# iammadab/zk

Measured on AMD Instinct MI355X. Metric: field-ops/sec (MLE fold, 2^24 evals, BN254 Fr) + sumcheck prover wall-clock, higher is better.
Workload: dtype u256 (8 x u32 Montgomery limbs, integer)

## Files before the change

include/zk_amd.h:

```cpp
#ifndef ZK_AMD_H
#define ZK_AMD_H

#include <stddef.h>
#include <stdint.h>

#ifdef __cplusplus
extern "C" {
#endif

#define ZK_AMD_ABI_VERSION 6

typedef enum zk_field {
    ZK_FIELD_BN254_FR = 0,
    ZK_FIELD_BLS12_381_FR = 1,
    ZK_FIELD_BLS12_377_FR = 2
} zk_field;

typedef enum zk_status {
    ZK_OK = 0,
    ZK_ERR_EVAL_LEN = -1,
    ZK_ERR_EVAL_ARITY = -2,
    ZK_ERR_EMPTY_PRODUCT = -3,
    ZK_ERR_ARITY_MISMATCH = -4,
    ZK_ERR_PANIC_INDEX = -5,
// ... 216 lines not shown
int32_t zk_merkle_n_vars(const zk_merkle *m, uint32_t *out);
int32_t zk_merkle_n_columns(const zk_merkle *m, uint32_t *out);
int32_t zk_merkle_root(zk_ctx *ctx, const zk_merkle *m, uint8_t out[32]);
int32_t zk_merkle_level(zk_ctx *ctx, const zk_merkle *m, uint32_t level, uint8_t *out);
int32_t zk_merkle_open(zk_ctx *ctx, const zk_merkle *m, const zk_mle *const *columns, uint32_t n_columns,
                       const uint64_t *indices, uint64_t n_queries, uint64_t *out_rows, uint8_t *out_paths);
int32_t zk_merkle_verify_host(int32_t field, const uint8_t root[32], uint32_t n_vars, uint32_t n_columns, uint64_t index,
                              const uint64_t *row, const uint8_t *path, int32_t *out_ok);

int32_t zk_fri_lde(zk_ctx *ctx, const zk_upoly *p, uint32_t log_n, const uint64_t shift[4], zk_mle **out);
int32_t zk_fri_fold(zk_ctx *ctx, const zk_mle *in, uint32_t log_arity, const uint64_t shift[4], const uint64_t beta[4], zk_mle *out);
int32_t zk_fri_proof_bytes(uint32_t log_degree, uint32_t log_blowup, uint32_t log_arity, uint32_t log_final, uint32_t n_queries, uint64_t *out);
int32_t zk_fri_prove(zk_ctx *ctx, const zk_upoly *p, uint32_t log_degree, uint32_t log_blowup, uint32_t log_arity, uint32_t log_final,
                     uint32_t n_queries, const uint64_t shift[4], const uint8_t seed[32], uint8_t *out_proof);
int32_t zk_fri_verify_host(int32_t field, uint32_t log_degree, uint32_t log_blowup, uint32_t log_arity, uint32_t log_final,
                           uint32_t n_queries, const uint64_t shift[4], const uint8_t seed[32], const uint8_t *proof, uint64_t proof_len,
                           int32_t *out_ok);

typedef struct zk_pcs zk_pcs;
int32_t zk_deep_quotient(zk_ctx *ctx, const zk_mle *const *columns, uint32_t n_columns, const uint64_t shift[4], const uint64_t z[4],
                         const uint64_t *values, const uint64_t alpha[4], zk_mle *out);
int32_t zk_pcs_commit(zk_ctx *ctx, const zk_upoly *const *polys, uint32_t k, uint32_t log_degree, uint32_t log_blowup, uint32_t log_arity,
                      const uint64_t shift[4], zk_pcs **out);
int32_t zk_pcs_free(zk_pcs *h);
int32_t zk_pcs_n_polys(const zk_pcs *h, uint32_t *out);
int32_t zk_pcs_root(zk_ctx *ctx, const zk_pcs *h, uint8_t out[32]);
int32_t zk_pcs_proof_bytes(uint32_t k, uint32_t log_degree, uint32_t log_blowup, uint32_t log_arity, uint32_t log_final, uint32_t n_queries,
                           uint64_t *out);
int32_t zk_pcs_open(zk_ctx *ctx, const zk_pcs *h, const uint64_t z[4], uint32_t log_final, uint32_t n_queries, const uint8_t seed[32],
                    uint64_t *out_values, uint8_t *out_proof);
int32_t zk_pcs_verify_host(int32_t field, uint32_t k, uint32_t log_degree, uint32_t log_blowup, uint32_t log_arity, uint32_t log_final,
                           uint32_t n_queries, const uint64_t shift[4], const uint8_t seed[32], const uint8_t root[32], const uint64_t z[4],
                           const uint64_t *values, const uint8_t *proof, uint64_t proof_len, int32_t *out_ok);

int32_t zk_bench_fold(zk_ctx *ctx, const zk_mle *t, const uint64_t r[4], zk_mle *out, int32_t reps, double *out_ms);
int32_t zk_bench_fold_samples(zk_ctx *ctx, const zk_mle *t, const uint64_t r[4], zk_mle *out, int32_t reps, int32_t group,
                              double *out_ms_each);
int32_t zk_bench_ntt(zk_ctx *ctx, const zk_mle *in, int32_t inverse, zk_mle *out, int32_t reps, double *out_ms);
int32_t zk_bench_upoly_interp(zk_ctx *ctx, const zk_upoly *xs, const zk_upoly *ys, int32_t reps, double *out_ms);
int32_t zk_bench_upoly_evaluate_many(zk_ctx *ctx, const zk_upoly *p, const zk_upoly *xs, int32_t path, int32_t reps, double *out_ms);
int32_t zk_bench_upoly_divrem(zk_ctx *ctx, const zk_upoly *a, const zk_upoly *b, int32_t path, int32_t reps, double *out_ms);
int32_t zk_bench_cmle(zk_ctx *ctx, int32_t op, const zk_mle *t, const zk_cmle *p, const uint64_t *point, uint64_t n_point, int32_t reps,
                      double *out_ms);
int32_t zk_bench_cmle_algebra(zk_ctx *ctx, int32_t op, const zk_cmle *a, const zk_cmle *b, const uint8_t *selectors,
                              const uint64_t *selector_lens, const uint64_t *values, uint64_t n_assign, int32_t reps, double *out_ms);
int32_t zk_bench_batch_inverse(zk_ctx *ctx, const zk_mle *t, zk_mle *out, int32_t path, int32_t reps, double *out_ms);
int32_t zk_bench_merkle(zk_ctx *ctx, const zk_mle *const *columns, uint32_t n_columns, int32_t path, int32_t reps, double *out_ms);
int32_t zk_bench_fri_fold(zk_ctx *ctx, const zk_mle *in, uint32_t log_arity, zk_mle *out, int32_t path, int32_t reps, double *out_ms);
int32_t zk_bench_deep_quotient(zk_ctx *ctx, const zk_mle *const *columns, uint32_t n_columns, zk_mle *out, int32_t reps, double *out_ms);
int32_t zk_bench_prove_partial(zk_ctx *ctx, zk_mle *const *factors, uint64_t k, uint32_t max_var_degree, const uint64_t sum[4],
                               int32_t reps, double *out_ms_each);
int32_t zk_bench_evaluate(zk_ctx *ctx, const zk_mle *t, const uint64_t *point, uint64_t n_point, int32_t reps, double *out_ms_each);
int32_t zk_bench_evaluate_device(zk_ctx *ctx, const zk_mle *t, const uint64_t *point, uint64_t n_point, int32_t reps, double *out_ms);
int32_t zk_bench_modmul(zk_ctx *ctx, int32_t variant, int32_t iters, double *out_modmul_per_s);
int32_t zk_bench_copy(zk_ctx *ctx, uint64_t bytes, int32_t reps, double *out_gbps);


#ifdef __cplusplus
}
#endif
#endif
```

zk_amd/_lib.py:

```python
import ctypes
import os
import re

_HERE = os.path.dirname(os.path.abspath(__file__))
_DEFAULT_LIB = os.path.join(_HERE, "libzk_amd.so")
LIB_PATH = os.environ.get("ZK_AMD_LIB") or _DEFAULT_LIB
LIB_OVERRIDDEN = os.path.realpath(LIB_PATH) != os.path.realpath(_DEFAULT_LIB)
HEADER_PATH = os.path.join(os.path.dirname(_HERE), "include", "zk_amd.h")
if LIB_OVERRIDDEN:
    import sys as _sys

    _root = os.path.realpath(os.path.dirname(_HERE))
    if not os.path.realpath(LIB_PATH).startswith(_root + os.sep):
        raise ImportError(f"ZK_AMD_LIB={LIB_PATH} is outside {_root}: refused (the override is for builds of this tree only)")
    print(f"zk_amd: ZK_AMD_LIB override active: loading {os.path.realpath(LIB_PATH)}", file=_sys.stderr, flush=True)

c = ctypes
u64p = c.POINTER(c.c_uint64)
u8p = c.POINTER(c.c_uint8)
vpp = c.POINTER(c.c_void_p)


class ZkError(Exception):

# ... 157 lines not shown
    "zk_fri_fold": [c.c_void_p, c.c_void_p, c.c_uint32, u64p, u64p, c.c_void_p],
    "zk_fri_proof_bytes": [c.c_uint32, c.c_uint32, c.c_uint32, c.c_uint32, c.c_uint32, u64p],
    "zk_fri_prove": [c.c_void_p, c.c_void_p, c.c_uint32, c.c_uint32, c.c_uint32, c.c_uint32, c.c_uint32, u64p, u8p, u8p],
    "zk_fri_verify_host": [c.c_int32, c.c_uint32, c.c_uint32, c.c_uint32, c.c_uint32, c.c_uint32, u64p, u8p, u8p, c.c_uint64, c.POINTER(c.c_int32)],
    "zk_deep_quotient": [c.c_void_p, vpp, c.c_uint32, u64p, u64p, u64p, u64p, c.c_void_p],
    "zk_pcs_commit": [c.c_void_p, vpp, c.c_uint32, c.c_uint32, c.c_uint32, c.c_uint32, u64p, vpp],
    "zk_pcs_free": [c.c_void_p],
    "zk_pcs_n_polys": [c.c_void_p, c.POINTER(c.c_uint32)],
    "zk_pcs_root": [c.c_void_p, c.c_void_p, u8p],
    "zk_pcs_proof_bytes": [c.c_uint32, c.c_uint32, c.c_uint32, c.c_uint32, c.c_uint32, c.c_uint32, u64p],
    "zk_pcs_open": [c.c_void_p, c.c_void_p, u64p, c.c_uint32, c.c_uint32, u8p, u64p, u8p],
    "zk_pcs_verify_host": [c.c_int32, c.c_uint32, c.c_uint32, c.c_uint32, c.c_uint32, c.c_uint32, c.c_uint32, u64p, u8p, u8p, u64p, u64p, u8p,
                           c.c_uint64, c.POINTER(c.c_int32)],
    "zk_ctx_device_alloc": [c.c_void_p, c.c_uint64, vpp],
    "zk_ctx_device_free": [c.c_void_p, c.c_void_p, c.c_uint64],
    "zk_ctx_memcpy_dtoh": [c.c_void_p, c.c_void_p, c.c_void_p, c.c_uint64],
    "zk_ctx_memcpy_htod": [c.c_void_p, c.c_void_p, c.c_void_p, c.c_uint64],
    "zk_sumcheck_verify_partial": [c.c_int32, c.c_uint64, c.c_uint32, u64p, u64p, u64p, u64p],
    "zk_sumcheck_verify": [c.c_void_p, vpp, c.c_uint64, c.c_uint64, c.c_uint32, u64p, u64p, c.POINTER(c.c_int32)],
    "zk_sumcheck_verify_partial_lengths": [c.c_int32, c.c_uint64, c.POINTER(c.c_uint32), u64p, u64p, u64p, u64p],
    "zk_sumcheck_verify_lengths": [c.c_void_p, vpp, c.c_uint64, c.c_uint64, c.POINTER(c.c_uint32), u64p, u64p,
                                   c.POINTER(c.c_int32)],
    "zk_sumcheck_prove_terms": [c.c_void_p, vpp, u64p, c.c_uint64, c.c_uint32, u64p, c.c_int32, u64p, u64p, u64p],
    "zk_eq_table": [c.c_void_p, u64p, c.c_uint64, vpp],
    "zk_circuit_create": [c.c_void_p, vpp],
    "zk_circuit_add_layer": [c.c_void_p, c.c_uint64, c.c_uint64, u8p, c.POINTER(c.c_uint32), c.POINTER(c.c_uint32)],
    "zk_circuit_free": [c.c_void_p],
    "zk_circuit_depth": [c.c_void_p, u64p],
    "zk_circuit_layer_dims": [c.c_void_p, c.c_uint64, u64p, u64p],
    "zk_circuit_proof_elems": [c.c_void_p, u64p],
    "zk_gkr_evaluate": [c.c_void_p, c.c_void_p, vpp],
    "zk_gkr_prove": [c.c_void_p, c.c_void_p, u8p, vpp, u64p],
    "zk_gkr_verify": [c.c_void_p, c.c_void_p, c.c_void_p, u8p, u64p],
    "zk_mle_mul_powers": [c.c_void_p, c.c_void_p, u64p, u64p],
    "zk_dft_across": [c.c_void_p, c.c_void_p, c.c_void_p, c.c_uint64, c.c_int32],
    "zk_ntt": [c.c_void_p, c.c_void_p, c.c_int32, c.c_void_p],
    "zk_fft_host": [c.c_void_p, u64p, c.c_uint64, u64p],
    "zk_ifft_host": [c.c_void_p, u64p, c.c_uint64, u64p],
    "zk_fft_internal_host": [c.c_void_p, u64p, c.c_uint64, u64p, u64p],
    "zk_bench_fold": [c.c_void_p, c.c_void_p, u64p, c.c_void_p, c.c_int32, c.POINTER(c.c_double)],
    "zk_bench_fold_samples": [c.c_void_p, c.c_void_p, u64p, c.c_void_p, c.c_int32, c.c_int32, c.POINTER(c.c_double)],
    "zk_bench_ntt": [c.c_void_p, c.c_void_p, c.c_int32, c.c_void_p, c.c_int32, c.POINTER(c.c_double)],
    "zk_bench_upoly_interp": [c.c_void_p, c.c_void_p, c.c_void_p, c.c_int32, c.POINTER(c.c_double)],
    "zk_bench_upoly_evaluate_many": [c.c_void_p, c.c_void_p, c.c_void_p, c.c_int32, c.c_int32, c.POINTER(c.c_double)],
    "zk_bench_upoly_divrem": [c.c_void_p, c.c_void_p, c.c_void_p, c.c_int32, c.c_int32, c.POINTER(c.c_double)],
    "zk_bench_cmle": [c.c_void_p, c.c_int32, c.c_void_p, c.c_void_p, u64p, c.c_uint64, c.c_int32, c.POINTER(c.c_double)],
    "zk_bench_cmle_algebra": [c.c_void_p, c.c_int32, c.c_void_p, c.c_void_p, u8p, u64p, u64p, c.c_uint64, c.c_int32, c.POINTER(c.c_double)],
    "zk_bench_batch_inverse": [c.c_void_p, c.c_void_p, c.c_void_p, c.c_int32, c.c_int32, c.POINTER(c.c_double)],
    "zk_bench_merkle": [c.c_void_p, vpp, c.c_uint32, c.c_int32, c.c_int32, c.POINTER(c.c_double)],
    "zk_bench_fri_fold": [c.c_void_p, c.c_void_p, c.c_uint32, c.c_void_p, c.c_int32, c.c_int32, c.POINTER(c.c_double)],
    "zk_bench_deep_quotient": [c.c_void_p, vpp, c.c_uint32, c.c_void_p, c.c_int32, c.POINTER(c.c_double)],
    "zk_bench_prove_partial": [c.c_void_p, c.POINTER(c.c_void_p), c.c_uint64, c.c_uint32, u64p, c.c_int32, c.POINTER(c.c_double)],
    "zk_bench_evaluate": [c.c_void_p, c.c_void_p, u64p, c.c_uint64, c.c_int32, c.POINTER(c.c_double)],
    "zk_bench_evaluate_device": [c.c_void_p, c.c_void_p, u64p, c.c_uint64, c.c_int32, c.POINTER(c.c_double)],
    "zk_bench_modmul": [c.c_void_p, c.c_int32, c.c_int32, c.POINTER(c.c_double)],
    "zk_bench_copy": [c.c_void_p, c.c_uint64, c.c_int32, c.POINTER(c.c_double)],
}
for _name, _args in _sig.items():
    if LIB_OVERRIDDEN and not hasattr(lib, _name):
        continue
    _f = getattr(lib, _name)
    _f.argtypes = _args
    _f.restype = c.c_int32


def lib_info():
    return {"path": os.path.realpath(LIB_PATH), "overridden_by_ZK_AMD_LIB": bool(LIB_OVERRIDDEN), "abi": int(lib.zk_abi_version())}
```

zk_amd/api.py:

```python
import numpy as np

from ._lib import ZkError, c, check, lib, u8p, u64p

BN254_FR, BLS12_381_FR, BLS12_377_FR = 0, 1, 2
FIELD_NAMES = {BN254_FR: "bn254_fr", BLS12_381_FR: "bls12_381_fr", BLS12_377_FR: "bls12_377_fr"}


def _p(a):
    return a.ctypes.data_as(u64p)


def _elems(x, n=None):
    a = np.ascontiguousarray(x, dtype=np.uint64).reshape(-1, 4)
    if n is not None and a.shape[0] != n:
        raise ValueError(f"expected {n} field elements, got {a.shape[0]}")
    return a


def modulus(field):
    out = np.zeros(4, dtype=np.uint64)
    check(lib.zk_field_modulus(field, _p(out)))
    return sum(int(v) << (64 * i) for i, v in enumerate(out))


# ... 164 lines not shown
        check(lib.zk_mle_interleave(shards[0].ctx._h, ptrs, len(shards), c.byref(h)))
        return cls(shards[0].ctx, h)

    @classmethod
    def alloc(cls, ctx, n_vars):
        h = c.c_void_p()
        check(lib.zk_mle_alloc(ctx._h, n_vars, c.byref(h)))
        return cls(ctx, h)

    @classmethod
    def random(cls, ctx, n_vars, seed, first_index=0):
        t = cls.alloc(ctx, n_vars)
        check(lib.zk_mle_fill_random(ctx._h, t._h, seed, first_index))
        return t

    def free(self):
        if getattr(self, "_h", None) and getattr(self.ctx, "_h", None):
            lib.zk_mle_free(self.ctx._h, self._h)
        self._h = None

    def __del__(self):
        self.free()

    def clone(self):
        h = c.c_void_p()
        check(lib.zk_mle_clone(self.ctx._h, self._h, c.byref(h)))
        return MultiLinearPolynomial(self.ctx, h)

    def split(self, world):
        hs = (c.c_void_p * max(int(world), 1))()
        check(lib.zk_mle_split(self.ctx._h, self._h, world, c.cast(hs, c.POINTER(c.c_void_p))))
        return [MultiLinearPolynomial(self.ctx, c.c_void_p(h)) for h in hs[:world]]

    def n_vars(self):
        n = c.c_uint64()
        check(lib.zk_mle_n_vars(self._h, c.byref(n)))
        return n.value

    def device_ptr(self):
        p = c.c_void_p()
        check(lib.zk_mle_device_ptr(self._h, c.byref(p)))
        return p.value

    def partial_evaluate(self, initial_var, assignments):
        a = _elems(assignments)
        h = c.c_void_p()
        check(lib.zk_mle_partial_evaluate(self.ctx._h, self._h, initial_var, _p(a), a.shape[0], c.byref(h)))
        return MultiLinearPolynomial(self.ctx, h)

    def fold_into(self, r, out):
        r = _elems(r, 1)
        check(lib.zk_mle_fold_into(self.ctx._h, self._h, _p(r), out._h))
        return out

    def bench_fold(self, r, out, reps):
        r = _elems(r, 1)
        ms = c.c_double()
        check(lib.zk_bench_fold(self.ctx._h, self._h, _p(r), out._h, reps, c.byref(ms)))
        return ms.value

    def bench_fold_samples(self, r, out, reps, group=1):
        r = _elems(r, 1)
        ms = np.zeros((reps + group - 1) // group, dtype=np.float64)
        check(lib.zk_bench_fold_samples(self.ctx._h, self._h, _p(r), out._h, reps, group, ms.ctypes.data_as(c.POINTER(c.c_double))))
        return ms

    def evaluate(self, assignments):
        a = _elems(assignments)
        out = np.zeros(4, dtype=np.uint64)
        check(lib.zk_mle_evaluate(self.ctx._h, self._h, _p(a), a.shape[0], _p(out)))
        return out

    def evaluation_slice(self):
        out = np.zeros((1 << self.n_vars(), 4), dtype=np.uint64)
        check(lib.zk_mle_download(self.ctx._h, self._h, _p(out)))
        return out

    def to_bytes_array(self, out=None):
        if out is None:
            out = np.empty(32 << self.n_vars(), dtype=np.uint8)
        want = 32 << self.n_vars()
        if not isinstance(out, np.ndarray) or out.dtype != np.uint8 or out.size != want:
            raise ValueError(f"to_bytes_array: out must be a numpy uint8 array of {want} bytes")
        if not out.flags["C_CONTIGUOUS"] or not out.flags["WRITEABLE"]:
            raise ValueError("to_bytes_array: out must be C-contiguous and writeable")
        check(lib.zk_mle_to_bytes(self.ctx._h, self._h, out.ctypes.data_as(u8p)))
        return out

    def to_bytes(self):
        return self.to_bytes_array().tobytes()

    def batch_inverse(self, shift=None, out=None, count_zeros=False):
        if out is None:
            out = MultiLinearPolynomial.alloc(self.ctx, self.n_vars())
        sv = None if shift is None else _elems(shift, 1)
        zeros = c.c_uint64()
        check(lib.zk_mle_batch_inverse(self.ctx._h, self._h, None if sv is None else _p(sv), out._h, c.byref(zeros) if count_zeros else None))
        return (out, zeros.value) if count_zeros else out

    def prefix_product(self, inclusive=False, out=None, want_total=False):
        if out is None:
            out = MultiLinearPolynomial.alloc(self.ctx, self.n_vars())
        total = np.zeros(4, dtype=np.uint64)
        check(lib.zk_mle_prefix_product(self.ctx._h, self._h, 1 if inclusive else 0, out._h, _p(total) if want_total else None))
        return (out, total) if want_total else out

# ... 806 lines not shown
```

zk_amd/csrc/capi.hip:

```cpp
#include <hip/hip_runtime.h>
#include <sched.h>

#include <algorithm>
#include <array>
#include <atomic>
#include <chrono>
#include <condition_variable>
#include <mutex>
#include <cstdio>
#include <map>
#include <new>
#include <set>
#include <string>
#include <thread>
#include <utility>
#include <vector>

#include "../../include/zk_amd.h"
#include "host_core.hpp"
#include "timing.hpp"
#include "copy_helpers.hpp"
#include "env.hpp"
#include "kernels.cuh"
#include "eval_kernels.cuh"
// ... 353 lines not shown
        return ZK_OK;
    }
    if (a->d == b->d) {
        *out = 1;
        return ZK_OK;
    }
    ZKCHK(use_device(c));
    uint32_t *d_flag = reinterpret_cast<uint32_t *>(c->d_sums);
    HIPCHK(hipMemsetAsync(d_flag, 0, 4, c->stream));
    const uint64_t n16 = (uint64_t)2 << a->n_vars;
    k_compare<<<grid_for(n16), kBlock, 0, c->stream>>>(reinterpret_cast<const uint4 *>(a->d), reinterpret_cast<const uint4 *>(b->d), n16, d_flag);
    HIPCHK(hipGetLastError());
    HIPCHK(hipMemcpyAsync(c->h_pinned, d_flag, 4, hipMemcpyDeviceToHost, c->stream));
    HIPCHK(hipStreamSynchronize(c->stream));
    *out = *reinterpret_cast<uint32_t *>(c->h_pinned) == 0 ? 1 : 0;
    return ZK_OK;
}
extern "C" int32_t zk_mle_device_ptr(const zk_mle *t, void **out) {
    if (!t || !out) return ZK_ERR_BAD_ARG;
    *out = t->d;
    return ZK_OK;
}

static int32_t launch_fold(zk_ctx *c, const uint64_t *in, uint64_t *out, uint64_t m, uint64_t initial_var, const Fe &r) {
    const uint64_t pairs = 1ull << (m - 1);
    const uint32_t pos = (uint32_t)(m - 1 - initial_var);
    if (initial_var == 0 && pairs >= 64) {
        uint64_t g = pairs / kBlock;
        if (g > 2 * kMaxGridStream) g = 2 * kMaxGridStream;
        k_fold_msb<<<(uint32_t)(g ? g : 1), kBlock, 0, c->stream>>>(in, out, pairs, c->fi->P, mul29_prepare(r, c->fi->P));
        HIPCHK(hipGetLastError());
        return ZK_OK;
    }
    if (pos >= 6 && in != out) {
        uint64_t g = pairs / kBlock;
        if (g > 2 * kMaxGridStream) g = 2 * kMaxGridStream;
        k_fold_run<<<(uint32_t)(g ? g : 1), kBlock, 0, c->stream>>>(in, out, pairs, pos, c->fi->P, mul29_prepare(r, c->fi->P));
        HIPCHK(hipGetLastError());
        return ZK_OK;
    }
    if (pos < 6 && pairs >= 64 && in != out) {
        uint64_t g = pairs / kBlock;
        if (g > 2 * kMaxGridStream) g = 2 * kMaxGridStream;
        k_fold_low<<<(uint32_t)(g ? g : 1), kBlock, 0, c->stream>>>(in, out, pairs, pos, c->fi->P, mul29_prepare(r, c->fi->P));
        HIPCHK(hipGetLastError());
        return ZK_OK;
    }
    uint64_t g = (pairs + kBlock - 1) / kBlock;
    if (g > kMaxGridStream) g = kMaxGridStream;
    k_fold<<<(uint32_t)(g ? g : 1), kBlock, 0, c->stream>>>(in, out, pairs, pos, c->fi->P, mul29_prepare(r, c->fi->P));
    HIPCHK(hipGetLastError());
    return ZK_OK;
}
static int32_t check_partial_args(uint64_t n_vars, uint64_t initial_var, uint64_t n_assign) {
    if (n_assign > n_vars) return ZK_ERR_PANIC_INDEX;
    for (uint64_t i = 0; i < n_assign; ++i) {
        const uint64_t nv = n_vars - i;
        if (nv == 0 || initial_var > nv - 1) return ZK_ERR_PANIC_INDEX;
    }
    return ZK_OK;
}

extern "C" int32_t zk_mle_partial_evaluate(zk_ctx *c, const zk_mle *t, uint64_t initial_var, const uint64_t *assignments,
                                           uint64_t n_assign, zk_mle **out) {
    if (!c || !t || !out || (!assignments && n_assign)) return ZK_ERR_BAD_ARG;
    if (t->ctx != c) return ZK_ERR_CONTEXT_MISMATCH;
    ZKCHK(check_partial_args(t->n_vars, initial_var, n_assign));
    ZKCHK(use_device(c));
    if (n_assign == 0) return zk_mle_clone(c, t, out);
    MleHolder res, tmp[2];
    ZKCHK(mle_alloc(c, t->n_vars - n_assign, res.put()));
    if (n_assign >= 2) ZKCHK(mle_alloc(c, t->n_vars - 1, tmp[0].put()));
    if (n_assign >= 3) ZKCHK(mle_alloc(c, t->n_vars - 2, tmp[1].put()));
    const uint64_t *src = t->d;
    for (uint64_t i = 0; i < n_assign; ++i) {
        uint64_t *dst = (i == n_assign - 1) ? res->d : tmp[i & 1]->d;
        ZKCHK(launch_fold(c, src, dst, t->n_vars - i, initial_var, fe_from_u64limbs(assignments + 4 * i)));
        src = dst;
    }
    *out = res.release();
    return ZK_OK;
}

extern "C" int32_t zk_mle_fold_into(zk_ctx *c, const zk_mle *t, const uint64_t r[4], zk_mle *out) {
    if (!c || !t || !r || !out) return ZK_ERR_BAD_ARG;
    if (t->ctx != c || out->ctx != c) return ZK_ERR_CONTEXT_MISMATCH;
    if (t->n_vars == 0) return ZK_ERR_PANIC_INDEX;
    if (out->n_vars != t->n_vars - 1) return ZK_ERR_BAD_ARG;
    ZKCHK(use_device(c));
    return launch_fold(c, t->d, out->d, t->n_vars, 0, fe_from_u64limbs(r));
}

int32_t zk::evaluate_device(zk_ctx *c, const zk_mle *t, const uint64_t *point, uint64_t *d_out_elem, uint32_t flag_seq) {
    const uint64_t n = t->n_vars;
    if (n == 0) {
        HIPCHK(hipMemcpyAsync(d_out_elem, t->d, 32, hipMemcpyDeviceToDevice, c->stream));
        return ZK_OK;
    }
    const FieldParams &P = c->fi->P;
    PoolBlock scratch[2];
    const uint64_t *src = t->d;
    uint64_t cur = n;
    static const bool bulk_low = !env_flag("ZK_EVAL_FOLDS");
    static const uint64_t stream_min = env_u64("ZK_EVAL_STREAM_MIN", 21, 0, 1000);
    for (int pass = 0; bulk_low && cur >= 8; ++pass) {
        static const uint64_t leave_env = env_u64("ZK_EVAL_STREAM_LEAVE", 0, 7, kEvalHighMax);
        const uint64_t stream_leave = leave_env ? leave_env : (cur <= 21 ? (uint64_t)8 : (uint64_t)9);
        const bool stream = cur >= stream_min && cur >= (uint64_t)kEvalStreamMin + stream_leave;
        uint64_t L = cur <= (uint64_t)kEvalLowMax ? cur : cur - 8;
        if (L > (uint64_t)kEvalLowMax) L = kEvalLowMax;
        if (L < (uint64_t)kEvalLowMin) L = kEvalLowMin;
        if (stream) L = cur - stream_leave < (uint64_t)kEvalStreamMax ? cur - stream_leave : (uint64_t)kEvalStreamMax;
        const uint64_t n_out = 1ull << (cur - L);
        uint64_t *dst = d_out_elem;
        if (L != cur) {
            const int b = pass & 1;
            if (!scratch[b] || scratch[b].bytes < n_out * 32) ZKCHK(scratch[b].alloc(c, (size_t)n_out * 32));
            dst = scratch[b].as();
        }
        const uint64_t H = cur - L;
        EvalHighPoint ph = {};
        static const int weight_mode = (int)env_u64("ZK_EVAL_WEIGHT", 3, 0, 3);
        if (H >= 1 && H <= (uint64_t)kEvalHighMax && (weight_mode & (stream ? 2 : 1))) {
            ph.n = (uint32_t)H;
            for (uint64_t p = 0; p < H; ++p) {
                const Fe r = fe_from_u64limbs(point + 4 * (H - 1 - p));
                for (int i = 0; i < 8; ++i) ph.r[p][i] = r.v[i];
            }
        }
        if (stream) {
            EvalStreamPoint sp = {};
// ... 564 lines not shown
    HIPCHK(hipMemcpyAsync(dst_dev, src_host, bytes, hipMemcpyHostToDevice, c->stream));
    HIPCHK(hipStreamSynchronize(c->stream));
    return ZK_OK;
}
extern "C" int32_t zk_ctx_device_alloc(zk_ctx *c, uint64_t bytes, void **out) {
    if (!c || !out) return ZK_ERR_BAD_ARG;
    ZKCHK(use_device(c));
    PoolBlock blk;
    ZKCHK(blk.alloc(c, bytes));
    *out = blk.release();
    return ZK_OK;
}
extern "C" int32_t zk_ctx_device_free(zk_ctx *c, void *ptr, uint64_t bytes) {
    if (!c) return ZK_ERR_BAD_ARG;
    pool_free(c, ptr, bytes);
    return ZK_OK;
}

extern "C" int32_t zk_bench_fold(zk_ctx *c, const zk_mle *t, const uint64_t r[4], zk_mle *out, int32_t reps, double *out_ms) {
    if (!c || !t || !r || !out || !out_ms || reps <= 0) return ZK_ERR_BAD_ARG;
    if (t->ctx != c || out->ctx != c) return ZK_ERR_CONTEXT_MISMATCH;
    if (t->n_vars == 0 || out->n_vars != t->n_vars - 1) return ZK_ERR_BAD_ARG;
    ZKCHK(use_device(c));
    const Fe rr = fe_from_u64limbs(r);
    return timed_span(c, 0, AfterWarm::kNoWait, reps, [&] { return launch_fold(c, t->d, out->d, t->n_vars, 0, rr); }, out_ms);
}
extern "C" int32_t zk_bench_fold_samples(zk_ctx *c, const zk_mle *t, const uint64_t r[4], zk_mle *out, int32_t reps, int32_t group,
                                         double *out_ms_each) {
    if (!c || !t || !r || !out || !out_ms_each || reps <= 0 || group <= 0 || reps > (1 << 20)) return ZK_ERR_BAD_ARG;
    if (t->ctx != c || out->ctx != c) return ZK_ERR_CONTEXT_MISMATCH;
    if (t->n_vars == 0 || out->n_vars != t->n_vars - 1) return ZK_ERR_BAD_ARG;
    ZKCHK(use_device(c));
    const Fe rr = fe_from_u64limbs(r);
    const int n_samples = (reps + group - 1) / group;
    if (n_samples > 65536) return ZK_ERR_BAD_ARG;
    PhaseEvents ev(c);
    ZKCHK(ev.create((size_t)n_samples - 1));
    DrainOnExit drain(c);
    ZKCHK(ev.begin());
    for (int i = 0; i < reps; ++i) {
        ZKCHK(launch_fold(c, t->d, out->d, t->n_vars, 0, rr));
        if (i + 1 == reps) ZKCHK(ev.end());
        else if ((i + 1) % group == 0) ZKCHK(ev.mark((size_t)(i / group)));
    }
    drain.armed = false;
    for (int i = 0; i < n_samples; ++i) {
        double ms = 0.0;
        ZKCHK(ev.span_ms((size_t)i, (size_t)i + 1, &ms));
        const int launches = i + 1 < n_samples ? group : reps - i * group;
        out_ms_each[i] = ms / launches;
    }
    return ZK_OK;
}
extern "C" int32_t zk_bench_evaluate(zk_ctx *c, const zk_mle *t, const uint64_t *point, uint64_t n_point, int32_t reps, double *out_ms_each) {
    if (!c || !t || !out_ms_each || reps <= 0) return ZK_ERR_BAD_ARG;
    uint64_t out[4];
    return wall_clock_each(c, reps, [&] { return zk_mle_evaluate(c, t, point, n_point, out); }, out_ms_each);
}
extern "C" int32_t zk_bench_evaluate_device(zk_ctx *c, const zk_mle *t, const uint64_t *point, uint64_t n_point, int32_t reps, double *out_ms) {
    if (!c || !t || !out_ms || reps <= 0 || (!point && n_point)) return ZK_ERR_BAD_ARG;
    if (t->ctx != c) return ZK_ERR_CONTEXT_MISMATCH;
    if (n_point != t->n_vars) return ZK_ERR_EVAL_ARITY;
    ZKCHK(use_device(c));
    return timed_span(c, 1, AfterWarm::kWait, reps, [&] { return evaluate_device(c, t, point, c->d_sums); }, out_ms);
}
extern "C" int32_t zk_bench_modmul(zk_ctx *c, int32_t variant, int32_t iters, double *out) {
    if (!c || !out || iters <= 0) return ZK_ERR_BAD_ARG;
    if (variant != 0 && variant != 1) return ZK_ERR_UNSUPPORTED;
    ZKCHK(use_device(c));
    const uint32_t blocks = 256 * 8;
    Fe seed = c->fi->two_adic_root;
    const Mul29 seed29 = mul29_prepare(seed, c->fi->P);
    k_bench_modmul<<<blocks, kBlock, 0, c->stream>>>(c->d_sums, 8, c->fi->P, seed, seed29, variant);
    double ms = 0.0;
    ZKCHK(timed_span(c, 0, AfterWarm::kNoWait, 1, [&] {
        k_bench_modmul<<<blocks, kBlock, 0, c->stream>>>(c->d_sums, iters, c->fi->P, seed, seed29, variant);
        return ZK_OK;
    }, &ms));
    *out = (double)blocks * kBlock * 2.0 * iters / (ms * 1e-3);
    return ZK_OK;
}
extern "C" int32_t zk_bench_copy(zk_ctx *c, uint64_t bytes, int32_t reps, double *out_gbps) {
    if (!c || !out_gbps || reps <= 0 || bytes < 16) return ZK_ERR_BAD_ARG;
    ZKCHK(use_device(c));
    RawBlock a_block, b_block;
    if (hipMalloc(a_block.put(), bytes) != hipSuccess || hipMalloc(b_block.put(), bytes) != hipSuccess) return ZK_ERR_ALLOC;
    uint4 *a = static_cast<uint4 *>(a_block.get()), *b = static_cast<uint4 *>(b_block.get());
    HIPCHK(hipMemsetAsync(a, 1, bytes, c->stream));
    const uint64_t n16 = bytes / 16;
    k_bench_copy<<<kMaxGrid, kBlock, 0, c->stream>>>(a, b, n16);
    double ms = 0.0;
    ZKCHK(timed_span(c, 0, AfterWarm::kNoWait, reps, [&] {
        k_bench_copy<<<kMaxGrid, kBlock, 0, c->stream>>>(a, b, n16);
        return ZK_OK;
    }, &ms));
    *out_gbps = 2.0 * (double)n16 * 16.0 / (ms * 1e-3) / 1e9;
    return ZK_OK;
}
```

zk_amd/csrc/field.cuh:

```cuda
#pragma once
#include <stdint.h>

#if defined(__HIPCC__)
#include <hip/hip_runtime.h>
#define ZK_HD __host__ __device__ __forceinline__
#define ZK_D __device__ __forceinline__
#else
#define ZK_HD inline
#define ZK_D inline
#endif

namespace zk {

struct FieldParams {
    uint32_t p[8];
    uint32_t r1[8];
    uint32_t r2[8];
    uint32_t inv;
    uint32_t bits;
    uint32_t p29[9];
    uint32_t inv29;
    uint32_t r2_29[9];
    uint32_t r2s_29[9];
};
// ... 417 lines not shown
        }
#pragma unroll
        for (int i = k - 8; i < 9; ++i) acc += (uint64_t)m[i] * P.p29[k - i];
        r[k - 9] = (uint32_t)acc & M;
        acc >>= 29;
    }
    r[8] = (uint32_t)acc;
    Fe s;
#pragma unroll
    for (int w = 0; w < 8; ++w) {
        const int bit = 32 * w, i = bit / 29, sh = bit - 29 * i;
        uint32_t v = r[i] >> sh;
        v |= r[i + 1] << (29 - sh);
        if (29 - sh + 29 < 32 && i + 2 < 9) v |= r[i + 2] << (58 - sh);
        s.v[w] = v;
    }
    if constexpr (LAZY) return s;
    Fe d, o;
    const uint32_t borrow = sub8(d.v, s.v, P.p);
#pragma unroll
    for (int i = 0; i < 8; ++i) o.v[i] = borrow ? s.v[i] : d.v[i];
    return o;
}
template <bool LAZY = false, bool TWO = false>
ZK_HD Fe fe_mul29_t(const Fe &a, const Mul29 &c, const FieldParams &P, const Fe *a2 = nullptr, const Mul29 *c2 = nullptr) {
    uint32_t x[9], y[9] = {0, 0, 0, 0, 0, 0, 0, 0, 0};
    split29(a.v, x);
    if constexpr (TWO) split29(a2->v, y);
    return mul29_core<LAZY, TWO>(x, y, c, P, c2);
}
ZK_HD void split29_shl5(const uint32_t a[8], uint32_t out[9]) {
    constexpr uint32_t M = (1u << 29) - 1;
    out[0] = (a[0] << 5) & M;
#pragma unroll
    for (int i = 1; i < 9; ++i) {
        const int bit = 29 * i - 5, w = bit >> 5, sh = bit & 31;
        uint32_t v = a[w] >> sh;
        if (sh > 3 && w + 1 < 8) v |= a[w + 1] << (32 - sh);
        out[i] = v & M;
    }
}
ZK_HD Fe fe_mul_tt(const Fe &a, const Fe &b, const FieldParams &P) {
    uint32_t x[9], y[9] = {0, 0, 0, 0, 0, 0, 0, 0, 0};
    Mul29 c;
    split29_shl5(a.v, x);
    split29(b.v, c.l);
    return mul29_core<false, false>(x, y, c, P);
}
ZK_HD Fe fe_dot2_29(const Fe &a, const Mul29 &c, const Fe &a2, const Mul29 &c2, const FieldParams &P) {
    return fe_mul29_t<false, true>(a, c, P, &a2, &c2);
}
ZK_HD Fe fe_mul29(const Fe &a, const Mul29 &c, const FieldParams &P) { return fe_mul29_t<false>(a, c, P); }

#if defined(__HIPCC__)
ZK_D Fe fe_load(const uint64_t *base, uint64_t idx) {
    const uint4 *q = reinterpret_cast<const uint4 *>(base + 4 * idx);
    uint4 a = q[0], b = q[1];
    Fe r = {{a.x, a.y, a.z, a.w, b.x, b.y, b.z, b.w}};
    return r;
}
ZK_D void fe_store(uint64_t *base, uint64_t idx, const Fe &r) {
    uint4 *q = reinterpret_cast<uint4 *>(base + 4 * idx);
    q[0] = make_uint4(r.v[0], r.v[1], r.v[2], r.v[3]);
    q[1] = make_uint4(r.v[4], r.v[5], r.v[6], r.v[7]);
}
#endif

}
```

zk_amd/csrc/host_field.hpp:

```cpp
#pragma once
#include <stdint.h>
#include <string.h>

#include "field.cuh"

namespace zk {

struct FieldInfo {
    FieldParams P;
    uint32_t two_adicity;
    uint32_t generator;
    Fe two_adic_root;
    bool ready;
};

inline const uint64_t *field_modulus_limbs(int field) {
    static const uint64_t M[3][4] = {
        {0x43e1f593f0000001ULL, 0x2833e84879b97091ULL, 0xb85045b68181585dULL, 0x30644e72e131a029ULL},
        {0xffffffff00000001ULL, 0x53bda402fffe5bfeULL, 0x3339d80809a1d805ULL, 0x73eda753299d7d48ULL},
        {0x0a11800000000001ULL, 0x59aa76fed0000001ULL, 0x60b44d1e5c37b001ULL, 0x12ab655e9a2ca556ULL},
    };
    return (field >= 0 && field < 3) ? M[field] : nullptr;
}

// ... 48 lines not shown
    int top = 7;
    while (top > 0 && P.p[top] == 0) --top;
    P.bits = 32 * top + (32 - __builtin_clz(P.p[top]));
    uint32_t v[8] = {1, 0, 0, 0, 0, 0, 0, 0}, d[8];
    for (int i = 0; i < 512; ++i) {
        uint32_t c = add8(v, v, v);
        uint32_t b = sub8(d, v, P.p);
        if (c | (b ^ 1u)) memcpy(v, d, 32);
        if (i == 255) memcpy(P.r1, v, 32);
    }
    memcpy(P.r2, v, 32);
    split29(P.p, P.p29);
    P.inv29 = P.inv & ((1u << 29) - 1);
    {
        Fe r2;
        memcpy(r2.v, P.r2, 32);
        const Mul29 k0 = mul29_prepare(r2, P);
        Fe r2s = r2;
        for (int i = 0; i < 5; ++i) r2s = fe_add(r2s, r2s, P);
        const Mul29 k1 = mul29_prepare(r2s, P);
        memcpy(P.r2_29, k0.l, sizeof k0.l);
        memcpy(P.r2s_29, k1.l, sizeof k1.l);
    }
    {
        const int rp_log = 257 - (int)P.bits;
        int lazy_log = 0;
        while ((1 << lazy_log) < kMaxLazy) ++lazy_log;
        const int top_log = lazy_log + 2 * (int)P.bits - 512;
        const uint64_t rp = rp_log >= 0 && rp_log < 32 ? (1ull << rp_log) : ~0ull;
        const uint64_t top = top_log < 0 ? 0 : (top_log < 32 ? (1ull << top_log) : ~0ull);
        if (rp_log < 0 || rp + 1 + top >= 32 || rp + 1 + top < rp) return nullptr;
    }
    I.two_adicity = adicity[field];
    I.generator = gen[field];
    uint32_t t[8], one[8] = {1, 0, 0, 0, 0, 0, 0, 0};
    sub8(t, P.p, one);
    for (uint32_t s = 0; s < I.two_adicity; ++s) {
        for (int i = 0; i < 7; ++i) t[i] = (t[i] >> 1) | (t[i + 1] << 31);
        t[7] >>= 1;
    }
    I.two_adic_root = fe_pow_limbs(fe_from_u32(I.generator, P), t, P);
    I.ready = true;
    return &I;
}

inline bool field_root_of_unity(const FieldInfo &I, uint32_t log_n, Fe &out) {
    if (log_n > I.two_adicity) return false;
    Fe w = I.two_adic_root;
    for (uint32_t i = log_n; i < I.two_adicity; ++i) w = fe_sqr(w, I.P);
    out = w;
    return true;
}

inline void fe_to_bytes_be(const Fe &a, const FieldParams &P, uint8_t out[32]) {
    Fe c = fe_to_canonical(a, P);
    for (int i = 0; i < 8; ++i)
        for (int b = 0; b < 4; ++b) out[31 - (4 * i + b)] = (uint8_t)(c.v[i] >> (8 * b));
}
inline Fe fe_from_be_bytes_mod_order(const uint8_t *bytes, size_t len, const FieldParams &P) {
    Fe acc = fe_zero();
    const Fe c256 = fe_from_u32(256, P);
    for (size_t i = 0; i < len; ++i) acc = fe_add(fe_mul(acc, c256, P), fe_from_u32(bytes[i], P), P);
    return acc;
}

}
```

zk_amd/csrc/kernels.cuh:

```cuda
#pragma once
#include "common.cuh"

namespace zk {

ZK_D uint64_t insert_zero_bit(uint64_t val, uint32_t pos) {
    const uint64_t low = val & ((1ull << pos) - 1ull);
    return ((val >> pos) << (pos + 1)) | low;
}

__global__ __launch_bounds__(kBlock) void k_fold(const uint64_t *in, uint64_t *out,
                                                 uint64_t pairs, uint32_t pos, FieldParams P, Mul29 r) {
    const uint64_t stride = (uint64_t)gridDim.x * kBlock;
    for (uint64_t j = (uint64_t)blockIdx.x * kBlock + threadIdx.x; j < pairs; j += stride) {
        const uint64_t l = insert_zero_bit(j, pos);
        const Fe lo = fe_load(in, l);
        const Fe hi = fe_load(in, l | (1ull << pos));
        const Fe d = fe_sub(lo, hi, P);
        fe_store(out, j, fe_sub(lo, fe_mul29(d, r, P), P));
    }
}

__global__ __launch_bounds__(kBlock) void k_fold_msb(const uint64_t *in, uint64_t *out, uint64_t half, FieldParams P, Mul29 r) {
    const uint32_t lane = threadIdx.x & 63;
    const bool odd = lane & 1;
    const uint64_t wave = ((uint64_t)blockIdx.x * kBlock + threadIdx.x) >> 6;
    const uint64_t nwaves = ((uint64_t)gridDim.x * kBlock) >> 6;
    const uint4 *in4 = reinterpret_cast<const uint4 *>(in);
    uint4 *out4 = reinterpret_cast<uint4 *>(out);
    for (uint64_t e0 = wave * 64; e0 < half; e0 += nwaves * 64) {
        const uint64_t c0 = 2 * e0 + lane;
        const uint4 la = nt_load16(in4 + c0), lb = nt_load16(in4 + c0 + 64);
        const uint4 ha = nt_load16(in4 + c0 + 2 * half), hb = nt_load16(in4 + c0 + 2 * half + 64);
        const Fe lo = pair_gather(la, lb, odd), hi = pair_gather(ha, hb, odd);
        const Fe o = fe_sub(lo, fe_mul29(fe_sub(lo, hi, P), r, P), P);
        uint4 oa, ob;
        pair_scatter(o, odd, oa, ob);
        nt_store16(oa, out4 + c0);
        nt_store16(ob, out4 + c0 + 64);
    }
}

__global__ __launch_bounds__(kBlock) void k_fold_run(const uint64_t *in, uint64_t *out, uint64_t pairs, uint32_t pos, FieldParams P, Mul29 r) {
    const uint32_t lane = threadIdx.x & 63;
    const bool odd = lane & 1;
    const uint64_t wave = ((uint64_t)blockIdx.x * kBlock + threadIdx.x) >> 6;
    const uint64_t nwaves = ((uint64_t)gridDim.x * kBlock) >> 6;
    const uint4 *in4 = reinterpret_cast<const uint4 *>(in);
    uint4 *out4 = reinterpret_cast<uint4 *>(out);
    const uint64_t span = 1ull << pos;
    for (uint64_t e0 = wave * 64; e0 < pairs; e0 += nwaves * 64) {
        const uint64_t lo0 = ((e0 >> pos) << (pos + 1)) | (e0 & (span - 1));
        const uint64_t cl = 2 * lo0 + lane, co = 2 * e0 + lane;
        const uint4 la = nt_load16(in4 + cl), lb = nt_load16(in4 + cl + 64);
        const uint4 ha = nt_load16(in4 + cl + 2 * span), hb = nt_load16(in4 + cl + 2 * span + 64);
        const Fe lo = pair_gather(la, lb, odd), hi = pair_gather(ha, hb, odd);
        const Fe o = fe_sub(lo, fe_mul29(fe_sub(lo, hi, P), r, P), P);
        uint4 oa, ob;
        pair_scatter(o, odd, oa, ob);
        nt_store16(oa, out4 + co);
        nt_store16(ob, out4 + co + 64);
    }
}

ZK_D Fe lane_pull(const Fe &v, uint32_t src_lane) {
    Fe r;
#pragma unroll
    for (int i = 0; i < 8; ++i) r.v[i] = (uint32_t)__builtin_amdgcn_ds_bpermute((int)(src_lane << 2), (int)v.v[i]);
    return r;
}
__global__ __launch_bounds__(kBlock) void k_fold_low(const uint64_t *in, uint64_t *out, uint64_t pairs, uint32_t pos, FieldParams P, Mul29 r) {
    const uint32_t lane = threadIdx.x & 63;
    const uint64_t wave = ((uint64_t)blockIdx.x * kBlock + threadIdx.x) >> 6;
    const uint64_t nwaves = ((uint64_t)gridDim.x * kBlock) >> 6;
    const uint32_t own = pair_owned(lane);
    const bool high = (own >> pos) & 1u;
    const uint32_t partner_own = own ^ (1u << pos);
    const uint32_t partner = ((partner_own & 31u) << 1) | (partner_own >> 5);
    const uint32_t want = own, want_half = want >> 5, want_low = want & 31u;
    const uint32_t src_own = (((want_low >> pos) << (pos + 1)) | (want_low & ((1u << pos) - 1u))) | (want_half << pos);
    const uint32_t src = ((src_own & 31u) << 1) | (src_own >> 5);
    for (uint64_t e0 = wave * 64; e0 < pairs; e0 += nwaves * 64) {
        const Fe a = run_load_nt(in + 4 * (2 * e0), lane), b = run_load_nt(in + 4 * (2 * e0 + 64), lane);
        const Fe got = lane_pull(high ? a : b, partner);
        const Fe lo = high ? got : a, hi = high ? b : got;
        const Fe o = fe_sub(lo, fe_mul29(fe_sub(lo, hi, P), r, P), P);
        run_store_nt(out + 4 * e0, lane, lane_pull(o, src));
    }
}

struct FoldChallenges {
    Mul29 r[3];
};
template <int V>
__global__ __launch_bounds__(kBlock) void k_fold_multi(const uint64_t *in, uint64_t *out, uint64_t n_out, FieldParams P, FoldChallenges ch) {
    const uint64_t stride = (uint64_t)gridDim.x * kBlock;
    for (uint64_t j = (uint64_t)blockIdx.x * kBlock + threadIdx.x; j < n_out; j += stride) {
        Fe x[1 << V];
#pragma unroll
        for (int c = 0; c < (1 << V); ++c) x[c] = fe_load(in, j + (uint64_t)c * n_out);
#pragma unroll
        for (int lvl = 0; lvl < V; ++lvl) {
#pragma unroll
            for (int c = 0; c < (1 << (V - 1 - lvl)); ++c)
                x[c] = fe_sub(x[c], fe_mul29(fe_sub(x[c], x[c + (1 << (V - 1 - lvl))], P), ch.r[lvl], P), P);
        }
        fe_store(out, j, x[0]);
    }
}

__global__ __launch_bounds__(kBlock) void k_eval_sum(const uint64_t *__restrict__ in, uint32_t n, FieldParams P, uint64_t *__restrict__ out,
                                                     volatile uint32_t *flag, uint32_t seq) {
    __shared__ uint32_t red[kBlock / 64][8];
    const uint32_t tid = threadIdx.x, lane = tid & 63;
    Fe acc = fe_zero();
    Fe x[16];
#pragma unroll
    for (int i = 0; i < 16; ++i)
        if (tid + 256u * i < n) x[i] = fe_load(in, tid + 256u * i);
#pragma unroll
    for (int i = 0; i < 16; ++i)
        if (tid + 256u * i < n) acc = fe_add(acc, x[i], P);
    acc = fe_wave_sum(acc, P);
    if (lane == 0) {
#pragma unroll
        for (int i = 0; i < 8; ++i) red[tid >> 6][i] = acc.v[i];
    }
    __syncthreads();
    if (tid == 0) {
        for (int wv = 1; wv < kBlock / 64; ++wv) {
            Fe o;
#pragma unroll
            for (int i = 0; i < 8; ++i) o.v[i] = red[wv][i];
            acc = fe_add(acc, o, P);
        }
        fe_store(out, 0, acc);
        if (flag) {
            __threadfence_system();
            *flag = seq;
        }
    }
}

// ... 277 lines not shown
```

Baseline: 194.6 billion.

## Fuse multi-variable partial evaluation into a single weighted dot-product fold kernel

Partial evaluation previously ran one fold kernel per assigned variable, and each pass read and wrote the whole intermediate table. It now groups 2 or 3 variables into one pass. Each output is computed as an eq-weight dot product over 4 or 8 inputs, accumulated in 29-bit limb columns with inline mad_u64 asm and finished with a single Montgomery reduction. The weights are read straight from the kernel-argument segment. This trades intermediate memory traffic and repeated reductions for heavier asm and more register pressure, and it adds a benchmark entry point.

```diff
diff --git a/include/zk_amd.h b/include/zk_amd.h
--- a/include/zk_amd.h
+++ b/include/zk_amd.h
@@ -292,6 +292,8 @@
                                int32_t reps, double *out_ms_each);
 int32_t zk_bench_evaluate(zk_ctx *ctx, const zk_mle *t, const uint64_t *point, uint64_t n_point, int32_t reps, double *out_ms_each);
 int32_t zk_bench_evaluate_device(zk_ctx *ctx, const zk_mle *t, const uint64_t *point, uint64_t n_point, int32_t reps, double *out_ms);
+int32_t zk_bench_partial_evaluate(zk_ctx *ctx, const zk_mle *t, uint64_t initial_var, const uint64_t *assignments, uint64_t n_assign,
+                                  int32_t reps, double *out_ms);
 int32_t zk_bench_modmul(zk_ctx *ctx, int32_t variant, int32_t iters, double *out_modmul_per_s);
 int32_t zk_bench_copy(zk_ctx *ctx, uint64_t bytes, int32_t reps, double *out_gbps);
 
diff --git a/zk_amd/_lib.py b/zk_amd/_lib.py
--- a/zk_amd/_lib.py
+++ b/zk_amd/_lib.py
@@ -233,6 +233,7 @@
     "zk_bench_deep_quotient": [c.c_void_p, vpp, c.c_uint32, c.c_void_p, c.c_int32, c.POINTER(c.c_double)],
     "zk_bench_prove_partial": [c.c_void_p, c.POINTER(c.c_void_p), c.c_uint64, c.c_uint32, u64p, c.c_int32, c.POINTER(c.c_double)],
     "zk_bench_evaluate": [c.c_void_p, c.c_void_p, u64p, c.c_uint64, c.c_int32, c.POINTER(c.c_double)],
+    "zk_bench_partial_evaluate": [c.c_void_p, c.c_void_p, c.c_uint64, u64p, c.c_uint64, c.c_int32, c.POINTER(c.c_double)],
     "zk_bench_evaluate_device": [c.c_void_p, c.c_void_p, u64p, c.c_uint64, c.c_int32, c.POINTER(c.c_double)],
     "zk_bench_modmul": [c.c_void_p, c.c_int32, c.c_int32, c.POINTER(c.c_double)],
     "zk_bench_copy": [c.c_void_p, c.c_uint64, c.c_int32, c.POINTER(c.c_double)],
diff --git a/zk_amd/api.py b/zk_amd/api.py
--- a/zk_amd/api.py
+++ b/zk_amd/api.py
@@ -240,6 +240,12 @@
         r = _elems(r, 1)
         check(lib.zk_mle_fold_into(self.ctx._h, self._h, _p(r), out._h))
         return out
+
+    def bench_partial_evaluate(self, initial_var, assignments, reps=5):
+        a = _elems(assignments)
+        ms = c.c_double()
+        check(lib.zk_bench_partial_evaluate(self.ctx._h, self._h, initial_var, _p(a), a.shape[0], reps, c.byref(ms)))
+        return ms.value
 
     def bench_fold(self, r, out, reps):
         r = _elems(r, 1)
diff --git a/zk_amd/csrc/capi.hip b/zk_amd/csrc/capi.hip
--- a/zk_amd/csrc/capi.hip
+++ b/zk_amd/csrc/capi.hip
@@ -429,6 +429,33 @@
     HIPCHK(hipGetLastError());
     return ZK_OK;
 }
+constexpr uint64_t kFoldMultiDefault = 3;
+static bool fold_multi_on(uint64_t group) {
+    static const uint64_t mode = env_u64("ZK_FOLD_MULTI", kFoldMultiDefault, 0, 3);
+    return group == 2 ? (mode & 1) != 0 : group == 3 ? (mode & 2) != 0 : false;
+}
+template <int A>
+static int32_t launch_fold_group_a(zk_ctx *c, const uint64_t *in, uint64_t *out, uint64_t m, uint64_t initial_var, const uint64_t *assignments) {
+    const FieldParams &P = c->fi->P;
+    Fe r[A], w[1 << A];
+    for (int i = 0; i < A; ++i) r[i] = fe_from_u64limbs(assignments + 4 * i);
+    fold_multi_weights(r, A, P, w);
+    FoldMultiArgs<A> args = {in, out, 1ull << (m - A), (uint32_t)(m - initial_var - A), P, {}};
+    for (int b = 0; b < (1 << A); ++b) {
+        const Mul29 p29 = mul29_prepare(w[b], P);
+        for (int i = 0; i < 9; ++i) args.w[b].l[i] = p29.l[i];
+    }
+    const uint64_t n_out = args.n_out;
+    static const uint64_t grid_cap = env_u64("ZK_FOLD_MULTI_MAX_GRID", 2 * kMaxGridStream, 1, 2 * kMaxGridStream);
+    uint64_t g = n_out / kBlock;
+    if (g > grid_cap) g = grid_cap;
+    k_fold_multi_run<A><<<(uint32_t)(g ? g : 1), kBlock, 0, c->stream>>>(args);
+    HIPCHK(hipGetLastError());
+    return ZK_OK;
+}
+static int32_t launch_fold_group(zk_ctx *c, const uint64_t *in, uint64_t *out, uint64_t m, uint64_t initial_var, const uint64_t *assignments, uint64_t g) {
+    return g == 3 ? launch_fold_group_a<3>(c, in, out, m, initial_var, assignments) : launch_fold_group_a<2>(c, in, out, m, initial_var, assignments);
+}
 static int32_t check_partial_args(uint64_t n_vars, uint64_t initial_var, uint64_t n_assign) {
     if (n_assign > n_vars) return ZK_ERR_PANIC_INDEX;
     for (uint64_t i = 0; i < n_assign; ++i) {
@@ -445,15 +472,27 @@
     ZKCHK(check_partial_args(t->n_vars, initial_var, n_assign));
     ZKCHK(use_device(c));
     if (n_assign == 0) return zk_mle_clone(c, t, out);
-    MleHolder res, tmp[2];
+    MleHolder res;
     ZKCHK(mle_alloc(c, t->n_vars - n_assign, res.put()));
-    if (n_assign >= 2) ZKCHK(mle_alloc(c, t->n_vars - 1, tmp[0].put()));
-    if (n_assign >= 3) ZKCHK(mle_alloc(c, t->n_vars - 2, tmp[1].put()));
+    PoolBlock tmp[2];
     const uint64_t *src = t->d;
-    for (uint64_t i = 0; i < n_assign; ++i) {
-        uint64_t *dst = (i == n_assign - 1) ? res->d : tmp[i & 1]->d;
-        ZKCHK(launch_fold(c, src, dst, t->n_vars - i, initial_var, fe_from_u64limbs(assignments + 4 * i)));
+    uint64_t m = t->n_vars;
+    int step = 0;
+    for (uint64_t i = 0; i < n_assign; ++step) {
+        const uint64_t left = n_assign - i;
+        uint64_t g = left < 3 ? left : 3;
+        while (g > 1 && !(fold_multi_on(g) && m - initial_var - g >= 6)) --g;
+        uint64_t *dst = res->d;
+        if (i + g != n_assign) {
+            PoolBlock &b = tmp[step & 1];
+            if (!b) ZKCHK(b.alloc(c, mle_block_bytes(m - g)));
+            dst = b.as();
+        }
+        if (g == 1) ZKCHK(launch_fold(c, src, dst, m, initial_var, fe_from_u64limbs(assignments + 4 * i)));
+        else ZKCHK(launch_fold_group(c, src, dst, m, initial_var, assignments + 4 * i, g));
         src = dst;
+        m -= g;
+        i += g;
     }
     *out = res.release();
     return ZK_OK;
@@ -1124,6 +1163,18 @@
     }
     return ZK_OK;
 }
+extern "C" int32_t zk_bench_partial_evaluate(zk_ctx *c, const zk_mle *t, uint64_t initial_var, const uint64_t *assignments, uint64_t n_assign,
+                                             int32_t reps, double *out_ms) {
+    if (!c || !t || !out_ms || reps <= 0 || !assignments || n_assign == 0) return ZK_ERR_BAD_ARG;
+    if (t->ctx != c) return ZK_ERR_CONTEXT_MISMATCH;
+    ZKCHK(check_partial_args(t->n_vars, initial_var, n_assign));
+    ZKCHK(use_device(c));
+    auto once = [&]() -> int32_t {
+        MleHolder o;
+        return zk_mle_partial_evaluate(c, t, initial_var, assignments, n_assign, o.put());
+    };
+    return timed_span(c, 1, AfterWarm::kWait, reps, once, out_ms);
+}
 extern "C" int32_t zk_bench_evaluate(zk_ctx *c, const zk_mle *t, const uint64_t *point, uint64_t n_point, int32_t reps, double *out_ms_each) {
     if (!c || !t || !out_ms_each || reps <= 0) return ZK_ERR_BAD_ARG;
     uint64_t out[4];
diff --git a/zk_amd/csrc/field.cuh b/zk_amd/csrc/field.cuh
--- a/zk_amd/csrc/field.cuh
+++ b/zk_amd/csrc/field.cuh
@@ -493,6 +493,89 @@
 }
 ZK_HD Fe fe_mul29(const Fe &a, const Mul29 &c, const FieldParams &P) { return fe_mul29_t<false>(a, c, P); }
 
+struct Dot29Cols {
+    uint64_t c[17];
+};
+ZK_HD void dot29_zero(Dot29Cols &a) {
+#pragma unroll
+    for (int k = 0; k < 17; ++k) a.c[k] = 0;
+}
+ZK_HD void dot29_mac(Dot29Cols &a, const uint32_t (&x)[9], const Mul29 &w) {
+#if defined(__HIP_DEVICE_COMPILE__) && !defined(ZK_NO_ASM)
+#define ZK_DM(C, X, W) "v_mad_u64_u32 %" #C ", vcc, %" #X ", %" #W ", %" #C "\n\t"
+    asm(ZK_DM(0, 13, 18) ZK_DM(1, 13, 19) ZK_DM(2, 13, 20) ZK_DM(3, 13, 21) ZK_DM(4, 13, 22) ZK_DM(5, 13, 23) ZK_DM(6, 13, 24) ZK_DM(7, 13, 25) ZK_DM(8, 13, 26)
+        ZK_DM(1, 14, 18) ZK_DM(2, 14, 19) ZK_DM(3, 14, 20) ZK_DM(4, 14, 21) ZK_DM(5, 14, 22) ZK_DM(6, 14, 23) ZK_DM(7, 14, 24) ZK_DM(8, 14, 25) ZK_DM(9, 14, 26)
+        ZK_DM(2, 15, 18) ZK_DM(3, 15, 19) ZK_DM(4, 15, 20) ZK_DM(5, 15, 21) ZK_DM(6, 15, 22) ZK_DM(7, 15, 23) ZK_DM(8, 15, 24) ZK_DM(9, 15, 25) ZK_DM(10, 15, 26)
+        ZK_DM(3, 16, 18) ZK_DM(4, 16, 19) ZK_DM(5, 16, 20) ZK_DM(6, 16, 21) ZK_DM(7, 16, 22) ZK_DM(8, 16, 23) ZK_DM(9, 16, 24) ZK_DM(10, 16, 25) ZK_DM(11, 16, 26)
+        ZK_DM(4, 17, 18) ZK_DM(5, 17, 19) ZK_DM(6, 17, 20) ZK_DM(7, 17, 21) ZK_DM(8, 17, 22) ZK_DM(9, 17, 23) ZK_DM(10, 17, 24) ZK_DM(11, 17, 25) ZK_DM(12, 17, 26)
+        : "+v"(a.c[0]), "+v"(a.c[1]), "+v"(a.c[2]), "+v"(a.c[3]), "+v"(a.c[4]), "+v"(a.c[5]), "+v"(a.c[6]), "+v"(a.c[7]), "+v"(a.c[8]),
+          "+v"(a.c[9]), "+v"(a.c[10]), "+v"(a.c[11]), "+v"(a.c[12])
+        : "v"(x[0]), "v"(x[1]), "v"(x[2]), "v"(x[3]), "v"(x[4]), "s"(w.l[0]), "s"(w.l[1]), "s"(w.l[2]), "s"(w.l[3]), "s"(w.l[4]), "s"(w.l[5]),
+          "s"(w.l[6]), "s"(w.l[7]), "s"(w.l[8])
+        : "vcc");
+    asm(ZK_DM(0, 12, 16) ZK_DM(1, 12, 17) ZK_DM(2, 12, 18) ZK_DM(3, 12, 19) ZK_DM(4, 12, 20) ZK_DM(5, 12, 21) ZK_DM(6, 12, 22) ZK_DM(7, 12, 23) ZK_DM(8, 12, 24)
+        ZK_DM(1, 13, 16) ZK_DM(2, 13, 17) ZK_DM(3, 13, 18) ZK_DM(4, 13, 19) ZK_DM(5, 13, 20) ZK_DM(6, 13, 21) ZK_DM(7, 13, 22) ZK_DM(8, 13, 23) ZK_DM(9, 13, 24)
+        ZK_DM(2, 14, 16) ZK_DM(3, 14, 17) ZK_DM(4, 14, 18) ZK_DM(5, 14, 19) ZK_DM(6, 14, 20) ZK_DM(7, 14, 21) ZK_DM(8, 14, 22) ZK_DM(9, 14, 23) ZK_DM(10, 14, 24)
+        ZK_DM(3, 15, 16) ZK_DM(4, 15, 17) ZK_DM(5, 15, 18) ZK_DM(6, 15, 19) ZK_DM(7, 15, 20) ZK_DM(8, 15, 21) ZK_DM(9, 15, 22) ZK_DM(10, 15, 23) ZK_DM(11, 15, 24)
+        : "+v"(a.c[5]), "+v"(a.c[6]), "+v"(a.c[7]), "+v"(a.c[8]), "+v"(a.c[9]), "+v"(a.c[10]), "+v"(a.c[11]), "+v"(a.c[12]), "+v"(a.c[13]),
+          "+v"(a.c[14]), "+v"(a.c[15]), "+v"(a.c[16])
+        : "v"(x[5]), "v"(x[6]), "v"(x[7]), "v"(x[8]), "s"(w.l[0]), "s"(w.l[1]), "s"(w.l[2]), "s"(w.l[3]), "s"(w.l[4]), "s"(w.l[5]), "s"(w.l[6]),
+          "s"(w.l[7]), "s"(w.l[8])
+        : "vcc");
+#undef ZK_DM
+#else
+#pragma unroll
+    for (int i = 0; i < 9; ++i)
+#pragma unroll
+        for (int j = 0; j < 9; ++j) a.c[i + j] += (uint64_t)x[i] * w.l[j];
+#endif
+}
+ZK_HD void dot29_normalise(Dot29Cols &a) {
+    constexpr uint64_t M = (1ull << 29) - 1;
+#pragma unroll
+    for (int k = 0; k < 16; ++k) {
+        a.c[k + 1] += a.c[k] >> 29;
+        a.c[k] &= M;
+    }
+}
+ZK_HD Fe dot29_redc(const Dot29Cols &a, const FieldParams &P) {
+    constexpr uint32_t M = (1u << 29) - 1;
+    uint32_t m[9], r[9];
+    uint64_t acc = 0;
+#pragma unroll
+    for (int k = 0; k < 9; ++k) {
+        acc += a.c[k];
+#pragma unroll
+        for (int i = 0; i < k; ++i) acc += (uint64_t)m[i] * P.p29[k - i];
+        m[k] = ((uint32_t)acc * P.inv29) & M;
+        acc += (uint64_t)m[k] * P.p29[0];
+        acc >>= 29;
+    }
+#pragma unroll
+    for (int k = 9; k < 17; ++k) {
+        acc += a.c[k];
+#pragma unroll
+        for (int i = k - 8; i < 9; ++i) acc += (uint64_t)m[i] * P.p29[k - i];
+        r[k - 9] = (uint32_t)acc & M;
+        acc >>= 29;
+    }
+    r[8] = (uint32_t)acc;
+    Fe s;
+#pragma unroll
+    for (int w = 0; w < 8; ++w) {
+        const int bit = 32 * w, i = bit / 29, sh = bit - 29 * i;
+        uint32_t v = r[i] >> sh;
+        v |= r[i + 1] << (29 - sh);
+        if (29 - sh + 29 < 32 && i + 2 < 9) v |= r[i + 2] << (58 - sh);
+        s.v[w] = v;
+    }
+    Fe d, o;
+    const uint32_t borrow = sub8(d.v, s.v, P.p);
+#pragma unroll
+    for (int i = 0; i < 8; ++i) o.v[i] = borrow ? s.v[i] : d.v[i];
+    return o;
+}
+
 #if defined(__HIPCC__)
 ZK_D Fe fe_load(const uint64_t *base, uint64_t idx) {
     const uint4 *q = reinterpret_cast<const uint4 *>(base + 4 * idx);
diff --git a/zk_amd/csrc/host_field.hpp b/zk_amd/csrc/host_field.hpp
--- a/zk_amd/csrc/host_field.hpp
+++ b/zk_amd/csrc/host_field.hpp
@@ -124,6 +124,16 @@
     return true;
 }
 
+inline void fold_multi_weights(const Fe *r, int A, const FieldParams &P, Fe *W ) {
+    W[0] = fe_one(P);
+    for (int i = 0; i < A; ++i)
+        for (int b = (1 << i) - 1; b >= 0; --b) {
+            const Fe hi = fe_mul(W[b], r[i], P);
+            W[2 * b] = fe_sub(W[b], hi, P);
+            W[2 * b + 1] = hi;
+        }
+}
+
 inline void fe_to_bytes_be(const Fe &a, const FieldParams &P, uint8_t out[32]) {
     Fe c = fe_to_canonical(a, P);
     for (int i = 0; i < 8; ++i)
diff --git a/zk_amd/csrc/kernels.cuh b/zk_amd/csrc/kernels.cuh
--- a/zk_amd/csrc/kernels.cuh
+++ b/zk_amd/csrc/kernels.cuh
@@ -1,4 +1,6 @@
 #pragma once
+#include <cstddef>
+
 #include "common.cuh"
 
 namespace zk {
@@ -88,6 +90,68 @@
     }
 }
 
+struct alignas(16) FoldWeight {
+    uint32_t l[12];
+};
+template <int A>
+struct FoldMultiArgs {
+    const uint64_t *in;
+    uint64_t *out;
+    uint64_t n_out;
+    uint32_t p_lo;
+    FieldParams P;
+    FoldWeight w[1 << A];
+};
+typedef const __attribute__((address_space(4))) u32x4_t *kernarg_quads_t;
+template <int A>
+__global__ __launch_bounds__(kBlock) void k_fold_multi_run(FoldMultiArgs<A> args) {
+    static_assert(A == 2 || A == 3, "dot29_redc takes at most eight products, normalised once after four");
+    static_assert(offsetof(FoldMultiArgs<A>, w) % 16 == 0 && sizeof(FoldWeight) == 48, "the weights are read as 16-byte words of the argument segment");
+    constexpr int N = 1 << A;
+    const uint64_t *in = args.in;
+    uint64_t *out = args.out;
+    const uint64_t n_out = args.n_out;
+    const uint32_t p_lo = args.p_lo;
+    const FieldParams &P = args.P;
+    const kernarg_quads_t wts = (kernarg_quads_t)__builtin_amdgcn_kernarg_segment_ptr() + offsetof(FoldMultiArgs<A>, w) / 16;
+    const uint32_t lane = threadIdx.x & 63;
+    const bool odd = lane & 1;
+    const uint64_t wave = ((uint64_t)blockIdx.x * kBlock + threadIdx.x) >> 6;
+    const uint64_t nwaves = ((uint64_t)gridDim.x * kBlock) >> 6;
+    const uint4 *in4 = reinterpret_cast<const uint4 *>(in);
+    uint4 *out4 = reinterpret_cast<uint4 *>(out);
+    const uint64_t span = 1ull << p_lo;
+    for (uint64_t e0 = wave * 64; e0 < n_out; e0 += nwaves * 64) {
+        const uint64_t b0 = ((e0 >> p_lo) << (p_lo + A)) | (e0 & (span - 1));
+        const uint64_t cl = 2 * b0 + lane, co = 2 * e0 + lane;
+        uint4 xa[N], xb[N];
+#pragma unroll
+        for (int b = 0; b < N; ++b) {
+            xa[b] = nt_load16(in4 + cl + 2 * span * b);
+            xb[b] = nt_load16(in4 + cl + 2 * span * b + 64);
+        }
+        Dot29Cols acc;
+        dot29_zero(acc);
+#pragma unroll
+        for (int b = 0; b < N; ++b) {
+            const Fe x = pair_gather(xa[b], xb[b], odd);
+            uint32_t l[9];
+            split29(x.v, l);
+            uint32_t at = 3 * b;
+            asm volatile("" : "+s"(at));
+            const u32x4_t w0 = wts[at], w1 = wts[at + 1], w2 = wts[at + 2];
+            const Mul29 w = {{w0.x, w0.y, w0.z, w0.w, w1.x, w1.y, w1.z, w1.w, w2.x}};
+            dot29_mac(acc, l, w);
+            if (b == 3 && N > 4) dot29_normalise(acc);
+        }
+        const Fe o = dot29_redc(acc, P);
+        uint4 oa, ob;
+        pair_scatter(o, odd, oa, ob);
+        nt_store16(oa, out4 + co);
+        nt_store16(ob, out4 + co + 64);
+    }
+}
+
 struct FoldChallenges {
     Mul29 r[3];
 };
```

Result: slower. 190.8 billion (-1.9%).
